# Photoroom/datago

Hardware: AMD Instinct MI355X
Metric: Mpixel/s device-resident JPEG decode+bucket-resize at 1/2/4/8 MI355X (higher is better)
Workload: dtype u8

## Files before the change

### datago_amd/csrc/kernels.hip

```cpp
#include <hip/hip_runtime.h>

#include "dg_destuff.h"
#include "dg_entropy.h"
#include "dg_pixel.h"
#include "dg_plane.h"
#include "kernels.h"

#pragma clang fp contract(off)

namespace dg {


__device__ __forceinline__ void load_tables(HuffTable *tabs, const HuffTable *pool, const ImageDesc &im) {
  const int words = (int)(sizeof(HuffTable) / 4);
  const int ns = im.nslots;
  for (int i = threadIdx.x; i < ns * words; i += blockDim.x) {
    int s = i / words, w = i - s * words;
    ((uint32_t *)&tabs[s])[w] = ((const uint32_t *)&pool[im.hslot[s]])[w];
  }
}

__device__ __forceinline__ uint32_t xcd_remap(uint32_t b, uint32_t n) {
  const uint32_t per = n >> 3, rem = n & 7, x = b & 7, l = b >> 3;
  return x * per + (x < rem ? x : rem) + l;
// ... 1020 lines not shown
    return (my * im.mcux + mx) * im.bpm + im.cfirst[c] + vy * chc + hx;
  };
  u32x4 r0 = {0, 0, 0, 0}, r1 = {0, 0, 0, 0};
  if (v0) r0 = *(const DG_GLOBAL u32x4 *)(coef + (size_t)block_index(bx0) * 64 + lane * 8);
  if (v1) r1 = *(const DG_GLOBAL u32x4 *)(coef + (size_t)block_index(bx1) * 64 + lane * 8);
  const DG_GLOBAL uint16_t *q = gp<const uint16_t>((uint64_t)(uintptr_t)qpool[im.qpool[c]].q);
  int32_t qc[8];
#pragma unroll
  for (int r = 0; r < 8; r++) qc[r] = q[r * 8 + lane];
  int32_t *bv0 = blkv + slot * LD, *bv1 = blkv + (slot + 32) * LD;
  {
    int16_t a[8], b[8];
    __builtin_memcpy(a, &r0, 16);
    __builtin_memcpy(b, &r1, 16);
#pragma unroll
    for (int i = 0; i < 8; i++) {
      const int n = kZigzagToNatural[lane * 8 + i];
      const int e = (n >> 3) * RS + (n & 7);
      bv0[e] = a[i];
      bv1[e] = b[i];
    }
  }
  __syncthreads();
  const bool zune = im.sem != 0;
  {
    int32_t v0[8], v1[8], w0[8], w1[8];
#pragma unroll
    for (int r = 0; r < 8; r++) {
      v0[r] = __mul24(bv0[r * RS + lane], qc[r]);
      v1[r] = __mul24(bv1[r * RS + lane], qc[r]);
    }
    idct_col(zune, v0, w0);
    idct_col(zune, v1, w1);
    __syncthreads();
#pragma unroll
    for (int r = 0; r < 8; r++) {
      bv0[r * RS + lane] = w0[r];
      bv1[r * RS + lane] = w1[r];
    }
  }
  __syncthreads();
  const uint32_t pst = cbw * 8;
  DG_GLOBAL uint8_t *plane = gp<uint8_t>(im.plane[c]) + (size_t)(by * 8 + lane) * pst;
  const bool rec = plane_is_rec(im, c);
  uint32_t pv[2][8];
#pragma unroll
  for (int h = 0; h < 2; h++) {
    const int32_t *w = (h ? bv1 : bv0) + lane * RS;
    const bool v = h ? v1 : v0;
    int32_t row[8];
    uint32_t px[8];
#pragma unroll
    for (int i = 0; i < 8; i++) row[i] = w[i];
    idct_row(zune, row, px);
    if (rec) {
      crec_clamp((int32_t)crec_lim(im, c) - 1 - (int32_t)((h ? bx1 : bx0) * 8), px, pv[h]);
      continue;
    }
    const uint32_t lo = pack4(px[0], px[1], px[2], px[3]), hi = pack4(px[4], px[5], px[6], px[7]);
    if (v) *(DG_GLOBAL u32x2 *)(plane + (size_t)(h ? bx1 : bx0) * 8) = u32x2{lo, hi};
  }
  if (!rec) return;
  __shared__ uint8_t efirst[kIdctBlocks * 8], elast[kIdctBlocks * 8];
#pragma unroll
  for (int h = 0; h < 2; h++) {
    const int i = slot + 32 * h;
    efirst[i * 8 + lane] = (uint8_t)pv[h][0];
    elast[i * 8 + lane] = (uint8_t)pv[h][7];
  }
  __syncthreads();
  DG_GLOBAL uint8_t *rrow = crec_row(im, c, by * 8 + lane);
#pragma unroll
  for (int h = 0; h < 2; h++) {
    if (!(h ? v1 : v0)) continue;
    const int i = slot + 32 * h;
    const uint32_t bx = h ? bx1 : bx0;
    const bool in_l = i > 0, in_r = i + 1 < (int)kIdctBlocks && bx + 1 < cbw;
    const uint32_t l = in_l ? elast[(i - 1) * 8 + lane] : pv[h][0];
    const uint32_t r = in_r ? efirst[(i + 1) * 8 + lane] : pv[h][7];
    store_crec_pair(rrow, bx, cbw, pv[h], l, r, in_l || bx == 0, in_r || bx + 1 == cbw);
  }
}

struct IdctLoc {
  uint32_t c, by, bx, bidx;
  bool v;
};
__device__ __forceinline__ bool idct_t_locate(const ImageDesc &im, uint32_t item, IdctLoc &L) {
  uint32_t c = 0;
  for (; c < im.ncomp; c++) {
    const uint32_t ck = (im.cbw[c] + kIdctBlocks - 1) / kIdctBlocks;
    const uint32_t n = im.cbh[c] * ck;
    if (item < n) break;
    item -= n;
  }
  if (c >= im.ncomp) return false;
  const uint32_t ck = (im.cbw[c] + kIdctBlocks - 1) / kIdctBlocks;
  const uint32_t by = item / ck, chunk = item - by * ck;
  const uint32_t cbw = im.cbw[c];
  const uint32_t bx = chunk * kIdctBlocks + threadIdx.x;
  const uint32_t chc = im.ch[c];
  uint32_t bidx;
  if (im.ncomp == 1) {
    bidx = by * cbw + bx;
  } else {
    const uint32_t my = by / im.cv[c], vy = by - my * im.cv[c];
    const uint32_t mx = chc == 1 ? bx : chc == 2 ? bx >> 1 : bx / chc, hx = bx - mx * chc;
    bidx = (my * im.mcux + mx) * im.bpm + im.cfirst[c] + vy * chc + hx;
  }
  L.c = c;
  L.by = by;
  L.bx = bx;
  L.v = bx < cbw;
  L.bidx = L.v ? bidx : 0u;
  return true;
}

__device__ __forceinline__ uint32_t idct_t_parts(const ImageDesc &im, const IdctLoc &L) {
  if (!L.v) return 0u;
  if (!im.ccnt) return 0xFFu;
  return gp<const uint8_t>(im.ccnt)[L.bidx];
}

__device__ __forceinline__ void idct_t_item(const ImageDesc &im, const IdctLoc &L, const u32x4 w[8],
                                            const QuantTable *__restrict__ qpool);

__global__ __launch_bounds__(64) void k_idct_t(const ImageDesc *__restrict__ imgs, const WgItem *__restrict__ list,
                                              const QuantTable *__restrict__ qpool) {
  const WgItem it = list[blockIdx.x];
  const ImageDesc &im = imgs[it.image];
  IdctLoc L;
  bool ok = idct_t_locate(im, it.item0, L);
  uint32_t np = ok ? idct_t_parts(im, L) : 0u;
#pragma nounroll
  for (uint32_t k = 0; k < kIdctItemStride && ok; k++) {
    u32x4 w[8];
    const DG_GLOBAL u32x4 *src = (const DG_GLOBAL u32x4 *)(gp<const int16_t>(im.coef) + (size_t)L.bidx * 64);
#pragma unroll
    for (uint32_t i = 0; i < 8; i++) w[i] = (np >> i) & 1u ? src[i] : u32x4{0, 0, 0, 0};
    IdctLoc N;
    const bool nok = k + 1 < kIdctItemStride && idct_t_locate(im, it.item0 + k + 1, N);
    const uint32_t nnp = nok ? idct_t_parts(im, N) : 0u;
    idct_t_item(im, L, w, qpool);
    L = N;
    ok = nok;
    np = nnp;
  }
}

__device__ __forceinline__ void idct_t_item(const ImageDesc &im, const IdctLoc &L, const u32x4 w[8],
                                            const QuantTable *__restrict__ qpool) {
  const uint32_t c = L.c, by = L.by, bx = L.bx;
  const bool v = L.v;
  const uint32_t lane = threadIdx.x, cbw = im.cbw[c];
  const bool zune = im.sem != 0;
  const DG_GLOBAL uint16_t *q = gp<const uint16_t>((uint64_t)(uintptr_t)qpool[im.qpool[c]].q);
  int32_t x[64];
  {
#pragma unroll
    for (int k = 0; k < 64; k++) {
      const uint32_t word = w[k >> 3][(k >> 1) & 3];
      const int32_t z = (int32_t)(int16_t)(k & 1 ? word >> 16 : word & 0xFFFFu);
      const int nat = kZigzagToNatural[k];
      x[nat] = __mul24(z, (int32_t)q[nat]);
    }
  }
#pragma unroll
  for (int col = 0; col < 8; col++) {
    int32_t in[8], o[8];
#pragma unroll
    for (int r = 0; r < 8; r++) in[r] = x[r * 8 + col];
    idct_col(zune, in, o);
#pragma unroll
    for (int r = 0; r < 8; r++) x[r * 8 + col] = o[r];
  }
  const bool rec = plane_is_rec(im, c);
  const int32_t e = rec ? (int32_t)crec_lim(im, c) - 1 - (int32_t)(bx * 8) : 7;
  DG_GLOBAL uint8_t *plane = gp<uint8_t>(im.plane[c]);
#pragma unroll
  for (int r = 0; r < 8; r++) {
    uint32_t px[8];
    idct_row(zune, x + r * 8, px);
    const uint32_t y = by * 8 + (uint32_t)r;
    if (!rec) {
      if (v)
        *(DG_GLOBAL u32x2 *)(plane + (size_t)y * (cbw * 8) + bx * 8) =
            u32x2{pack4(px[0], px[1], px[2], px[3]), pack4(px[4], px[5], px[6], px[7])};
      continue;
    }
    uint32_t vv[8];
    crec_clamp(e, px, vv);
    const uint32_t l = (uint32_t)__shfl_up((int)vv[7], 1), rr = (uint32_t)__shfl_down((int)vv[0], 1);
    if (v) {
      const bool have_l = lane > 0 || bx == 0, have_r = (lane + 1 < 64u && bx + 1 < cbw) || bx + 1 == cbw;
      store_crec_pair(crec_row(im, c, y), bx, cbw, vv, lane > 0 ? l : vv[0], bx + 1 < cbw ? rr : vv[7], have_l,
                      have_r);
    }
  }
}


__global__ __launch_bounds__(256) void k_idct_list(const ImageDesc *__restrict__ imgs,
                                                   const QuantTable *__restrict__ qpool,
                                                   const BatchFlags *__restrict__ flags) {
  constexpr int LD = 72, RS = 9;
  __shared__ int32_t blkv[32 * LD];
  const uint32_t n = flags->idct_late < flags->idct_cap ? flags->idct_late : flags->idct_cap;
  const DG_GLOBAL uint32_t *list = gp<const uint32_t>(flags->idct_list);
  const int t = threadIdx.x, slot = t >> 3, lane = t & 7;
  int32_t *bv = blkv + slot * LD;
  for (uint32_t base = blockIdx.x * 32; base < n; base += gridDim.x * 32) {
    const uint32_t e = base + (uint32_t)slot;
    const bool act = e < n;
    const uint32_t ii = act ? list[2 * e] : 0u, idx = act ? list[2 * e + 1] : 0u;
    const ImageDesc &im = imgs[ii];
    uint32_t c = 0, by = 0, bx = 0;
    if (act) block_pos(im, idx, c, by, bx);
    if (act) {
      const u32x4 r0 = *(const DG_GLOBAL u32x4 *)(gp<const int16_t>(im.coef) + (size_t)idx * 64 + lane * 8);
      int16_t a[8];
      __builtin_memcpy(a, &r0, 16);
#pragma unroll
      for (int i = 0; i < 8; i++) {
        const int nn = kZigzagToNatural[lane * 8 + i];
        bv[(nn >> 3) * RS + (nn & 7)] = a[i];
      }
    }
    __syncthreads();
    int32_t w[8];
    if (act) {
      const DG_GLOBAL uint16_t *q = gp<const uint16_t>((uint64_t)(uintptr_t)qpool[im.qpool[c]].q);
      int32_t v[8];
#pragma unroll
      for (int r = 0; r < 8; r++) v[r] = bv[r * RS + lane] * (int32_t)q[r * 8 + lane];
      idct_col(im.sem != 0, v, w);
    }
    __syncthreads();
    if (act) {
#pragma unroll
      for (int r = 0; r < 8; r++) bv[r * RS + lane] = w[r];
    }
    __syncthreads();
    if (act) {
      int32_t row[8];
      uint32_t px[8];
#pragma unroll
      for (int i = 0; i < 8; i++) row[i] = bv[lane * RS + i];
      idct_row(im.sem != 0, row, px);
      store_plane_row8(im, c, by * 8 + lane, bx, px);
    }
    __syncthreads();
  }
}


template <class P>
__device__ __forceinline__ void upsample8(P pl, uint32_t stride, uint32_t hr, uint32_t vr,
                                          uint32_t dsw, uint32_t dsh, uint32_t x0, uint32_t y, int32_t o[8],
                                          bool rec = false) {
  if (rec) {
    const uint32_t c0 = x0 >> 1;
    int32_t cs[6];
    const bool fancy = dsw > 2;
    if (vr == 1 || !fancy) {
      load_crec6(pl, stride, vr == 1 ? y : y >> 1, c0, cs);
      if (!fancy) {
#pragma unroll
        for (int k = 0; k < 8; k++) o[k] = cs[1 + (k >> 1)];
        return;
      }
#pragma unroll
      for (int k = 0; k < 4; k++) {
        const int32_t a = cs[k + 1] * 3;
        o[2 * k] = (a + cs[k] + 1) >> 2;
        o[2 * k + 1] = (a + cs[k + 2] + 2) >> 2;
      }
      return;
    }
    const uint32_t r = y >> 1;
// ... 2006 lines not shown
```

### datago_amd/csrc/dg_entropy.h

```cpp
#pragma once
#include "dg_pixel.h"
#include "dg_plane.h"
#include "dg_types.h"

namespace dg {

DG_HD int32_t huff_extend(int32_t v, int32_t s) { return v < (1 << (s - 1)) ? v - (1 << s) + 1 : v; }

DG_HD uint32_t bswap32(uint32_t x) {
  return (x >> 24) | ((x >> 8) & 0xFF00u) | ((x << 8) & 0xFF0000u) | (x << 24);
}

DG_HD uint32_t ds_word_index(uint32_t w, uint32_t lsw) {
  const uint32_t s = w >> lsw, j = w & ((1u << lsw) - 1u);
  return ((((s >> 6) << lsw) + j) << 6) + (s & 63u);
}
DG_HD uint64_t ds_words_alloc(uint32_t nsub, uint32_t lsw) {
  const uint32_t margin = ((1024u >> 5) >> lsw) + 2u;
  return ((uint64_t)((nsub + margin + 63u) / 64u) << lsw) * 64;
}

constexpr uint32_t kBwBuf = 6;

struct BitWin {
  const DG_GLOBAL uint32_t *w;
  uint64_t win;
  uint32_t base;
  uint32_t lsw;
  uint32_t nbuf;
  uint32_t buf[kBwBuf];
};

DG_HD uint32_t bw_word(const BitWin &b, uint32_t i) { return b.w[ds_word_index(i, b.lsw)]; }

DG_HD void bw_fill(BitWin &b) {
  const uint32_t nw = (b.base >> 5) + 2u;
#pragma unroll
  for (uint32_t k = 0; k < kBwBuf; k++) b.buf[k] = bw_word(b, nw + k);
  b.nbuf = kBwBuf;
}

DG_HD void bw_init(BitWin &b, const DG_GLOBAL uint8_t *stream, uint32_t lsw, uint32_t pos) {
  b.w = (const DG_GLOBAL uint32_t *)stream;
  b.lsw = lsw;
  uint32_t i = pos >> 5;
  b.base = i << 5;
  b.win = ((uint64_t)bswap32(bw_word(b, i)) << 32) | bswap32(bw_word(b, i + 1));
  bw_fill(b);
}

DG_HD void bw_refill(BitWin &b) {
#if defined(DG_DEVICE)
  if (__ballot(b.nbuf == 0u)) bw_fill(b);
#else
  if (b.nbuf == 0u) bw_fill(b);
#endif
}

DG_HD uint32_t bw_peek(const BitWin &b, uint32_t pos) { return (uint32_t)((b.win << (pos - b.base)) >> 32); }

DG_HD void bw_shift(BitWin &b, uint32_t pos) {
  const bool adv = pos - b.base >= 32u;
  b.win = adv ? (b.win << 32) | bswap32(b.buf[0]) : b.win;
  b.base += adv ? 32u : 0u;
#pragma unroll
  for (uint32_t k = 0; k + 1 < kBwBuf; k++) b.buf[k] = adv ? b.buf[k + 1] : b.buf[k];
  b.nbuf -= adv ? 1u : 0u;
}

DG_HD void bw_seek(BitWin &b, uint32_t pos) {
  if (pos - b.base >= 32u) bw_init(b, (const DG_GLOBAL uint8_t *)b.w, b.lsw, pos);
}

template <class T>
DG_HD uint32_t huff_lookup(const T &t, uint32_t bits) {
  uint32_t e = t.lut[bits >> (32 - kLutBits)];
  if (!(e & 0x8000u) && e) return e;
  if (e & 0x8000u) {
    uint32_t e2 = t.sub[e & (kMaxSubTables - 1)][(bits >> (32 - 16)) & ((1u << kSubBits) - 1)];
    return e2 ? e2 : (16u << 8);
  }
  uint32_t pk = bits >> 16;
  for (int32_t l = kLutBits + 1; l <= 16; l++)
    if (pk < t.lim[l]) return ((uint32_t)l << 8) | t.vals[(t.valoff[l] + (int32_t)(pk >> (16 - l))) & 255];
  return 16u << 8;
}

template <class T>
DG_HD uint32_t huff_decode(const T &t, uint32_t bits) {
  const uint32_t e = t.lut[bits >> (32 - kLutBits)];
  if (e != 0u && !(e & 0x8000u)) return e;
  return huff_lookup(t, bits);
}

DG_HD int32_t huff_value(uint32_t bits, uint32_t len, uint32_t size) {
  const uint32_t raw = (uint32_t)((uint64_t)(bits << len) >> (32u - size));
  const uint32_t half = (1u << size) >> 1;
  return raw < half ? (int32_t)raw - (int32_t)((1u << size) - 1u) : (int32_t)raw;
}

DG_HD uint32_t huff_next_z(uint32_t z, uint32_t sym) {
  const uint32_t size = sym & 15u, run = sym >> 4;
  const uint32_t zac = (size == 0u && run != 15u) ? 64u : z + run + 1u;
  return z == 0u ? 1u : zac;
}

#ifndef DG_MULTI_BITS
#define DG_MULTI_BITS 11
#endif
constexpr uint32_t kMultiBits = DG_MULTI_BITS;
constexpr uint32_t kMultiLuts = 3;

template <class TAB>
DG_HD uint32_t multi_entry(const TAB &t, uint32_t pfx) {
  const uint32_t bits = pfx << (32u - kMultiBits);
  uint32_t o = 0, adv = 0, eob = 0;
  while (o < kMultiBits) {
    const uint32_t e = huff_lookup(t, bits << o);
    const uint32_t len = e >> 8, sym = e & 0xFFu, size = sym & 15u, run = sym >> 4;
    if (len == 0u || len >= 16u || o + len + size > kMultiBits) break;
    if (size == 0u && run != 15u) {
      o += len;
      eob = 1;
      break;
    }
    const uint32_t nadv = adv + (size == 0u ? 16u : run + 1u);
    if (nadv > 64u) break;
    adv = nadv;
    o += len + size;
    if (adv == 64u) break;
  }
  return o | (adv << 4) | (eob << 11);
}

DG_HD uint32_t multi_next_z(uint32_t m, uint32_t z) {
  const uint32_t c = m & 15u, adv = (m >> 4) & 127u, eob = (m >> 11) & 1u;
  const bool ok = c != 0u && z != 0u && (eob ? z + adv < 64u : z + adv <= 64u);
  return ok ? (eob ? 64u : z + adv) : 0xFFFFFFFFu;
}

#if defined(DG_STEP_STATS) && !defined(DG_DEVICE)
struct StepStats {
  uint64_t lead_steps, range_steps, chained, over32;
};
inline StepStats g_step_stats = {0, 0, 0, 0};
#define DG_STEP_STAT(field, n) (g_step_stats.field += (n))
#else
#define DG_STEP_STAT(field, n) ((void)0)
#endif

#ifndef DG_CHAIN_DC
#define DG_CHAIN_DC 1
#endif
DG_HD void multi_chain(const uint16_t *mt, uint32_t mi, uint32_t bits, uint32_t chain, bool open, uint32_t ev,
                       uint32_t &used, uint32_t &pos, uint32_t &zn) {
#pragma unroll
  for (uint32_t x = 0; x < 3u; x++) {
    if (x >= chain) break;
    const uint32_t bx = used < 32u ? bits << used : 0u;
    const uint32_t m = (open && mi != 3u) ? (uint32_t)mt[(mi << kMultiBits) | (bx >> (32u - kMultiBits))] : 0u;
    const uint32_t c = m & 15u;
    const uint32_t zx = multi_next_z(m, zn);
    const bool tk = zx != 0xFFFFFFFFu && pos + c <= ev && used + c <= 32u;
    pos += tk ? c : 0u;
    used += tk ? c : 0u;
    zn = tk ? zx : zn;
    DG_STEP_STAT(chained, tk ? 1u : 0u);
  }
}

template <int NC>
struct RangeAccN {
  uint32_t out;
  uint32_t m, n;
  int32_t dc[NC];
};
using RangeAcc = RangeAccN<3>;
template <class T>
struct NoDeduce {
  typedef T type;
};

struct WriteCtxBase {
  int16_t *blk;
  uint32_t sw = 0;
  DG_GLOBAL int16_t *coef;
  uint32_t seg, nin;
  uint32_t blocks_per_seg, total_blocks;
  int32_t cur;
  uint32_t zs;
#if defined(DG_DEVICE)
  DG_GLOBAL uint8_t *cnt = nullptr;
  int16_t *wave_blk;
  uint32_t stride;
  uint32_t *tab;
  const ImageDesc *im;
  const int32_t *qt;
  const uint8_t *n2z;
  BatchFlags *flags;
  uint32_t img;
#endif
};
template <int NC>
struct WriteCtxN : WriteCtxBase {
  int32_t pred[NC];
};
using WriteCtx = WriteCtxN<3>;

DG_HD int32_t wc_index(const WriteCtxBase &w, uint32_t in_seg) {
  if (w.blocks_per_seg && in_seg >= w.blocks_per_seg) return -1;
  uint64_t g = (uint64_t)(w.blocks_per_seg ? w.seg : 0) * w.blocks_per_seg + in_seg;
  return g < w.total_blocks ? (int32_t)g : -1;
}

template <bool MS>
DG_HD int32_t wc_index_ms(const ImageDesc &im, const WriteCtxBase &w, uint32_t in_seg) {
  const int32_t g = wc_index(w, in_seg);
  if (MS && g >= 0 && im.ms.role == kMsScan) return (int32_t)ms_index(im.ms, (uint32_t)g);
  return g;
}

DG_HD void wc_begin(WriteCtxBase &w, int32_t idx, uint32_t zs) {
  w.cur = idx;
  w.zs = zs;
#if defined(DG_DEVICE)
  u32x4 *p = (u32x4 *)w.blk;
  const u32x4 zero = {0u, 0u, 0u, 0u};
#pragma unroll
  for (int i = 0; i < 8; i++) p[i] = zero;
#else
  for (int i = 0; i < 64; i++) w.blk[i] = 0;
#endif
}

DG_HD void wc_flush(WriteCtxBase &w, uint32_t ze) {
  if (w.cur < 0) return;
  DG_GLOBAL int16_t *dst = w.coef + (size_t)w.cur * 64;
  if (w.zs == 0 && ze == 64) {
#if defined(DG_DEVICE)
    const u32x4 *s4 = (const u32x4 *)w.blk;
    DG_GLOBAL u32x4 *d4 = (DG_GLOBAL u32x4 *)dst;
#pragma unroll
    for (int i = 0; i < 8; i++) d4[i] = s4[i ^ (w.sw >> 3)];
#else
    for (int i = 0; i < 64; i++) dst[i] = w.blk[i ^ w.sw];
#endif
  } else {
    for (uint32_t i = w.zs; i < ze; i++) dst[i] = w.blk[i ^ w.sw];
  }
#if defined(DG_DEVICE)
  if (w.cnt) w.cnt[w.cur] = 0xFFu;
#endif
  w.cur = -1;
}

#if defined(DG_DEVICE)
__device__ __forceinline__ void wc_list_late(WriteCtxBase &w, int32_t idx) {
  if (!w.im || idx < 0) return;
  const uint32_t e = atomicAdd(&w.flags->idct_late, 1u);
  if (e < w.flags->idct_cap) {
    uint32_t *l = (uint32_t *)(uintptr_t)w.flags->idct_list;
    l[2 * e] = w.img;
    l[2 * e + 1] = (uint32_t)idx;
  }
}

__device__ __forceinline__ void wc_coop_flush(WriteCtxBase &w, bool pending) {
  const uint64_t pm = __ballot(pending);
  if (!pm) return;
  const uint64_t am = __ballot(1);
  if (pending) {
    const uint32_t rank = __builtin_amdgcn_mbcnt_hi((uint32_t)(pm >> 32), __builtin_amdgcn_mbcnt_lo((uint32_t)pm, 0u));
    w.tab[rank] = __lane_id();
    w.tab[64 + rank] = (uint32_t)w.cur;
  }
  __builtin_amdgcn_wave_barrier();
  const uint32_t wr = __builtin_amdgcn_mbcnt_hi((uint32_t)(am >> 32), __builtin_amdgcn_mbcnt_lo((uint32_t)am, 0u));
  const uint32_t na = (uint32_t)__popcll(am), nb = (uint32_t)__popcll(pm), nc = 8u * nb;
  const u32x4 zero = {0u, 0u, 0u, 0u};
  if (w.im && na >= 8) {
    const ImageDesc &im = *w.im;
    const bool zune = im.sem != 0;
    const uint32_t groups = na >> 3, g = wr >> 3, part = wr & 7u;
    for (uint32_t k0 = 0; k0 < nb; k0 += groups) {
      const uint32_t k = k0 + g;
      const bool act = g < groups && k < nb;
      const int32_t idx = act ? (int32_t)w.tab[64 + k] : -1;
      const uint32_t own = act ? w.tab[k] & 255u : 0u;
      int16_t *b = w.wave_blk + own * w.stride;
      const uint32_t osw = w.stride == 64u ? ((own >> 1) & 7u) << 3 : 0u;
      const bool live = act && idx >= 0;
      uint32_t c = 0, by = 0, bx = 0;
      if (live) block_pos(im, (uint32_t)idx, c, by, bx);
      int32_t ws[8];
      if (live) {
        int32_t v[8];
#pragma unroll
        for (int r = 0; r < 8; r++) v[r] = (int32_t)b[w.n2z[r * 8 + part] ^ osw] * w.qt[c * 64 + r * 8 + part];
        idct_col(zune, v, ws);
      }
      __builtin_amdgcn_wave_barrier();
      if (live) {
#pragma unroll
        for (int r = 0; r < 8; r++) b[r * 8 + part] = (int16_t)ws[r];
      }
      __builtin_amdgcn_wave_barrier();
      if (act) {
        u32x4 *row4 = (u32x4 *)b + part;
        if (live) {
          const u32x4 rv = *row4;
          int16_t h[8];
          __builtin_memcpy(h, &rv, 16);
          int32_t row[8];
          uint32_t px[8];
#pragma unroll
          for (int i = 0; i < 8; i++) row[i] = h[i];
          idct_row(zune, row, px);
          store_plane_row8(im, c, by * 8 + part, bx, px);
        }
        *row4 = zero;
      }
      __builtin_amdgcn_wave_barrier();
    }
    return;
  }
  for (uint32_t c = wr; c < nc; c += na) {
    const uint32_t k = c >> 3, part = c & 7u;
    const int32_t idx = (int32_t)w.tab[64 + k];
    const uint32_t own = w.tab[k] & 255u;
    u32x4 *src = (u32x4 *)(w.wave_blk + own * w.stride) + (w.stride == 64u ? part ^ ((own >> 1) & 7u) : part);
    const u32x4 v = *src;
    const bool nz = (v.x | v.y | v.z | v.w) != 0u;
    if (idx >= 0 && (nz || !w.cnt)) *(DG_GLOBAL u32x4 *)(w.coef + (size_t)idx * 64 + part * 8) = v;
    if (w.cnt && nz) atomicOr(&w.tab[k], 256u << part);
    *src = zero;
    if (part == 0) wc_list_late(w, idx);
  }
  __builtin_amdgcn_wave_barrier();
  if (w.cnt && wr < nb) {
    const int32_t idx = (int32_t)w.tab[64 + wr];
    if (idx >= 0) w.cnt[idx] = (uint8_t)(w.tab[wr] >> 8);
  }
  __builtin_amdgcn_wave_barrier();
}

__device__ __forceinline__ void wc_flush_zero(WriteCtxBase &w, uint32_t ze) {
  wc_flush(w, ze);
  u32x4 *p = (u32x4 *)w.blk;
  const u32x4 zero = {0u, 0u, 0u, 0u};
#pragma unroll
  for (int i = 0; i < 8; i++) p[i] = zero;
}
#endif

template <bool COOP>
DG_HD void wc_end_block(WriteCtxBase &w, bool &pending) {
#if defined(DG_DEVICE)
  if (COOP) {
    if (w.zs == 0) {
      pending = true;
    } else {
      const int32_t idx = w.cur;
      wc_flush_zero(w, 64);
      wc_list_late(w, idx);
    }
    return;
  }
#endif
  (void)pending;
  wc_flush(w, 64);
}
template <bool COOP>
DG_HD void wc_partial(WriteCtxBase &w, uint32_t ze) {
#if defined(DG_DEVICE)
  if (COOP) {
    wc_flush_zero(w, ze);
    return;
  }
#endif
  wc_flush(w, ze);
}

struct StageCtx {
  DG_GLOBAL uint32_t *base;
  uint32_t on;
  uint32_t n, started;
  uint32_t g0, g1, g2, g3;
};
DG_HD uint32_t stage_coef(uint32_t zz, uint32_t j, int32_t v) {
  return (zz << 25) | ((j & 0x1FFFu) << 12) | ((uint32_t)v & 0xFFFu);
}
DG_HD uint32_t stage_marker(uint32_t owned, uint32_t z, uint32_t j) {
  return 0x80000000u | (owned << 30) | ((z & 63u) << 24) | ((j & 0x1FFFu) << 11);
}
DG_HD DG_GLOBAL uint32_t *stage_range(uint64_t stage, uint32_t cap, uint32_t s) {
  return (DG_GLOBAL uint32_t *)(uintptr_t)stage + ((((size_t)(s >> 6) * cap) << 6) + (s & 63u)) * 4;
}
DG_HD void stage_push(StageCtx &c, uint32_t e) {
  const uint32_t k = c.n & 3u;
  c.g0 = k == 0 ? e : c.g0;
  c.g1 = k == 1 ? e : c.g1;
  c.g2 = k == 2 ? e : c.g2;
  c.g3 = k == 3 ? e : c.g3;
  c.n++;
  if (k == 3) {
    DG_GLOBAL uint32_t *p = c.base + (size_t)((c.n >> 2) - 1) * 256;
// ... 153 lines not shown
  if (WRITE) {
    w->cur = -1;
    if (z > 0) wc_begin(*w, w->nin > 0 ? wc_index_ms<MS>(im, *w, w->nin - 1) : -1, z);
  }
  auto next_event = [&]() -> uint32_t {
    uint32_t e = a1 < mpos ? a1 : mpos;
    return (k < nck && cpos < e) ? cpos : e;
  };
  const bool multi = !WRITE && !stage && mt != nullptr;
  uint32_t mi = 3u;
  auto block_tables = [&](const TAB *&tdc, const TAB *&tac) {
    tdc = &tabs[(slotmap >> ((comp << 1) << 2)) & 15u];
    tac = &tabs[(slotmap >> (((comp << 1) | 1u) << 2)) & 15u];
    mi = multi ? (acm >> (2u * comp)) & 3u : 3u;
  };
  const TAB *tdc, *tac;
  block_tables(tdc, tac);
  uint32_t ev = next_event();
  for (;;) {
#if defined(DG_DEVICE)
    if (WRITE && COOP) {
      wc_coop_flush(*w, pending);
      pending = false;
    }
#endif
    if (pos >= ev) {
      if (pos >= mpos) {
        bool owned = mpos < a1;
        if (WRITE && z > 0) wc_partial<COOP>(*w, z);
        if (stage) stage_push(*stg, stage_marker(owned ? 1u : 0u, z, stg->started));
        pos = mpos;
        r = 0;
        z = 0;
        comp = cbits & 3u;
        block_tables(tdc, tac);
        if (owned) {
          acc.m++;
          acc.n = 0;
          setn(acc.dc, 0);
          if (WRITE) {
            w->seg++;
            w->nin = 0;
            setn(w->pred, 0);
          }
        }
        midx++;
        mpos = midx < im.nmk ? mk[midx] : kInf;
        bw_seek(b, pos);
      }
      if (k < nck && cpos < a1 && pos >= cpos) {
        uint32_t rel = pos - cpos;
        uint32_t st = pack_state(rel > 255 ? 255 : rel, r, z);
        DG_GLOBAL CkptN<NC> &c = ck[k];
        if (merge && c.st == st) {
          if (c.m) {
            acc.m += c.m;
            acc.n = c.n;
            cpyn<NC>(acc.dc, c.dc);
          } else {
            acc.n += c.n;
            accn<NC>(acc.dc, c.dc);
          }
          acc.out = old_out;
          merged = true;
          break;
        }
        c.st = st;
        c.m = acc.m;
        c.n = acc.n;
        cpyn<NC>(c.dc, acc.dc);
        k++;
        cpos += kCkptBits;
      }
      if (pos >= a1) break;
      ev = next_event();
    }
    bw_refill(b);
    const uint32_t bits = bw_peek(b, pos);
    const bool isdc = (z == 0);
    const uint32_t e = huff_decode(*(isdc ? tdc : tac), bits);
    const uint32_t len = e >> 8, sym = e & 0xFFu;
    const uint32_t size = sym & 15u;
    const uint32_t run = isdc ? 0u : (sym >> 4);
    const int32_t v = huff_value(bits, len, size);
    uint32_t zm = 0xFFFFFFFFu, mc = 0;
    if (!WRITE) {
      const uint32_t m = (mi != 3u && !isdc) ? (uint32_t)mt[(mi << kMultiBits) | (bits >> (32u - kMultiBits))] : 0u;
      mc = m & 15u;
      zm = pos + mc <= ev ? multi_next_z(m, z) : 0xFFFFFFFFu;
    }
    const bool take_m = zm != 0xFFFFFFFFu;
    const uint32_t p0 = pos;
    pos += take_m ? mc : len + size;
    const int32_t vdc = isdc ? v : 0;
    acc.n += isdc ? 1u : 0u;
    addn(acc.dc, comp, vdc);
    if (stage) {
      if (isdc) {
        stg->started++;
        if (v) stage_push(*stg, stage_coef(0, stg->started, v));
      } else if (size && z + run < 64) {
        stage_push(*stg, stage_coef(z + run, stg->started, v));
      }
    }
    if (WRITE) {
      addn(w->pred, comp, vdc);
      if (isdc) {
        if (COOP) {
          w->cur = wc_index_ms<MS>(im, *w, w->nin);
          w->zs = 0;
        } else {
          wc_begin(*w, wc_index_ms<MS>(im, *w, w->nin), 0);
        }
        w->nin++;
      }
      const uint32_t zz = z + run;
      if (isdc || (size && zz < 64u)) w->blk[zz ^ w->sw] = (int16_t)(isdc ? seln(w->pred, comp) : v);
    }
    uint32_t zn = take_m ? zm : huff_next_z(z, sym);
    if (pair && !stage && (WRITE || !take_m)) {
      uint32_t used = len + size;
      bool open = isdc || !(size == 0u && run != 15u);
#pragma unroll
      for (uint32_t x = 0; x < 3u; x++) {
        if (x >= pair) break;
        const uint32_t bx = used < 32u ? bits << used : 0u;
        const uint32_t ex = huff_decode(*tac, bx);
        const uint32_t lx = ex >> 8, sx = ex & 0xFFu, zx = sx & 15u;
        const bool tk = open && zn < 64u && pos < ev && used + lx + zx <= 32u;
        if (tk) {
          if (WRITE) {
            const uint32_t zz2 = zn + (sx >> 4);
            if (zx && zz2 < 64u) w->blk[zz2 ^ w->sw] = (int16_t)huff_value(bx, lx, zx);
          }
          pos += lx + zx;
          used += lx + zx;
          zn = huff_next_z(zn, sx);
        }
        open = tk && !(zx == 0u && (sx >> 4) != 15u);
      }
    }
    if (!WRITE && chain) {
      uint32_t used = pos - p0;
      multi_chain(mt, mi, bits, chain, DG_CHAIN_DC || !isdc, ev, used, pos, zn);
    }
    if (!WRITE) {
      DG_STEP_STAT(range_steps, 1u);
      DG_STEP_STAT(over32, pos - p0 > 32u ? 1u : 0u);
    }
    bw_shift(b, pos);
    const bool bend = zn >= 64u;
    if (WRITE && bend) wc_end_block<COOP>(*w, pending);
    z = bend ? 0u : zn;
    r = bend ? (r + 1u == bpm ? 0u : r + 1u) : r;
    comp = (cbits >> (2u * r)) & 3u;
    block_tables(tdc, tac);
  }
  if (WRITE && z > 0) wc_partial<COOP>(*w, z);
  if (stage) stage_finish(*stg);
  if (!merged) {
    uint32_t rel = pos - a1;
    acc.out = pack_state(rel > 255 ? 255 : rel, r, z);
  }
  for (uint32_t j = 0; j < k; j++) {
    DG_GLOBAL CkptN<NC> &c = ck[j];
    if (acc.m > c.m) {
      c.m = acc.m - c.m;
      c.n = acc.n;
      cpyn<NC>(c.dc, acc.dc);
    } else {
      c.m = 0;
      c.n = acc.n - c.n;
      rsubn<NC>(c.dc, acc.dc);
    }
  }
}

template <class TAB>
struct SyncChain {
  BitWin b;
  uint32_t pos, r, z, comp, mi, ev;
  uint32_t phase;
  uint32_t a0, a1, mpos, midx, k, cpos, nck;
  uint32_t in;
  const TAB *tdc, *tac;
  RangeAcc acc;
  DG_GLOBAL Ckpt *ck;
};

template <class TAB>
DG_HD void schain_tables(SyncChain<TAB> &c, const ImageDesc &im, const TAB *tabs, const uint16_t *mt, uint32_t acm) {
  c.tdc = &tabs[(im.slotmap >> ((c.comp << 1) << 2)) & 15u];
  c.tac = &tabs[(im.slotmap >> (((c.comp << 1) | 1u) << 2)) & 15u];
  c.mi = mt ? (acm >> (2u * c.comp)) & 3u : 3u;
}

template <class TAB>
DG_HD void schain_range(SyncChain<TAB> &c, const ImageDesc &im, const TAB *tabs, const DG_GLOBAL uint8_t *stream,
                        const DG_GLOBAL uint32_t *mk, const uint16_t *mt, uint32_t acm, bool fresh) {
  c.phase = 1;
  c.acc.m = 0;
  c.acc.n = 0;
  c.acc.dc[0] = c.acc.dc[1] = c.acc.dc[2] = 0;
  c.r = st_r(c.in);
  c.z = st_z(c.in);
  if (c.a0 >= im.ds_bits) {
    c.acc.out = pack_state(0, 0, 0);
    c.phase = 2;
    c.ev = kInf;
    c.comp = (im.comp_bits >> (2 * c.r)) & 3u;
    schain_tables(c, im, tabs, mt, acm);
    if (fresh) {
      c.pos = 0;
      bw_init(c.b, stream, im.ds_lsw, 0);
    }
    return;
  }
  c.pos = c.a0 + st_rel(c.in);
  c.mpos = im.nmk ? first_marker(mk, im.nmk, c.a0, c.midx) : kInf;
  if (fresh) bw_init(c.b, stream, im.ds_lsw, c.pos < c.a1 ? c.pos : c.a0);
  c.comp = (im.comp_bits >> (2 * c.r)) & 3u;
  schain_tables(c, im, tabs, mt, acm);
  c.k = 0;
  c.cpos = c.a0 + kCkptBits;
  const uint32_t e = c.a1 < c.mpos ? c.a1 : c.mpos;
  c.ev = (c.k < c.nck && c.cpos < e) ? c.cpos : e;
}

template <class TAB>
DG_HD void schain_begin(SyncChain<TAB> &c, const ImageDesc &im, const TAB *tabs, const DG_GLOBAL uint8_t *stream,
                        const DG_GLOBAL uint32_t *mk, uint32_t s, uint32_t lead, bool active, DG_GLOBAL Ckpt *ck,
// ... 183 lines not shown
```

Baseline: 140,500.

## Hoist per-image IDCT geometry into scalar registers and cache quant table

The k_idct_t kernel now reads the image descriptor through the constant address space and packs each component's geometry into wave-uniform values via readfirstlane, so they sit in scalar registers. Successive work items are reached by stepping a position incrementally instead of searching again with divisions on every item. The quant table is loaded once into registers through scalar loads and reloaded only when the quant slot changes, replacing per-element global 16-bit loads. The intent is to cut vector memory traffic and integer overhead in the IDCT loop, at the cost of more registers and hand-written crec row addressing that must match crec_row.

```diff
diff --git a/datago_amd/csrc/kernels.hip b/datago_amd/csrc/kernels.hip
--- a/datago_amd/csrc/kernels.hip
+++ b/datago_amd/csrc/kernels.hip
@@ -1126,79 +1126,163 @@
   }
 }
 
-struct IdctLoc {
-  uint32_t c, by, bx, bidx;
-  bool v;
+#define DG_CONST __attribute__((address_space(4)))
+
+struct IdctComp {
+  uint32_t cbw, cbh;
+  uint32_t lim;
+  uint32_t ch, cv, cfirst;
+  bool rec;
+  uint32_t qslot;
+  uint64_t plane;
 };
-__device__ __forceinline__ bool idct_t_locate(const ImageDesc &im, uint32_t item, IdctLoc &L) {
-  uint32_t c = 0;
-  for (; c < im.ncomp; c++) {
-    const uint32_t ck = (im.cbw[c] + kIdctBlocks - 1) / kIdctBlocks;
-    const uint32_t n = im.cbh[c] * ck;
-    if (item < n) break;
+struct IdctGeo {
+  uint32_t dims[4];
+  uint32_t info[4];
+  uint64_t plane[4];
+  uint32_t qslots[2];
+  uint32_t ncomp, mcux, bpm;
+  uint64_t coef, ccnt;
+  bool zune;
+};
+struct IdctPos {
+  uint32_t c, chunk, my, vy;
+  bool ok;
+};
+
+__device__ __forceinline__ uint32_t uni(uint32_t v) { return (uint32_t)__builtin_amdgcn_readfirstlane((int)v); }
+__device__ __forceinline__ uint64_t uni64(uint64_t v) { return (uint64_t)uni((uint32_t)(v >> 32)) << 32 | uni((uint32_t)v); }
+
+template <class T>
+__device__ __forceinline__ T idct_t_pick(uint32_t c, T a0, T a1, T a2, T a3) {
+  return c >= 2 ? (c == 3 ? a3 : a2) : (c == 1 ? a1 : a0);
+}
+__device__ __forceinline__ IdctComp idct_t_comp(const IdctGeo &g, uint32_t c) {
+  IdctComp r;
+  const uint32_t dims = idct_t_pick(c, g.dims[0], g.dims[1], g.dims[2], g.dims[3]);
+  const uint32_t info = idct_t_pick(c, g.info[0], g.info[1], g.info[2], g.info[3]);
+  r.cbw = dims & 0xFFFFu;
+  r.cbh = dims >> 16;
+  r.ch = info & 7u;
+  r.cv = (info >> 3) & 7u;
+  r.cfirst = (info >> 6) & 0x1FFu;
+  r.rec = (info >> 15) & 1u;
+  r.lim = g.zune ? r.cbw * 8 : info >> 16;
+  r.qslot = ((c & 2u ? g.qslots[1] : g.qslots[0]) >> (16 * (c & 1u))) & 0xFFFFu;
+  r.plane = idct_t_pick(c, g.plane[0], g.plane[1], g.plane[2], g.plane[3]);
+  return r;
+}
+
+__device__ __forceinline__ IdctPos idct_t_locate(const IdctGeo &g, uint32_t item) {
+  IdctPos p = {0, 0, 0, 0, false};
+  for (; p.c < g.ncomp; p.c++) {
+    const IdctComp cc = idct_t_comp(g, p.c);
+    const uint32_t ck = (cc.cbw + kIdctBlocks - 1) / kIdctBlocks, n = cc.cbh * ck;
+    if (item < n) {
+      const uint32_t by = item / ck;
+      p.chunk = item - by * ck;
+      p.my = by / cc.cv;
+      p.vy = by - p.my * cc.cv;
+      p.ok = true;
+      break;
+    }
     item -= n;
   }
-  if (c >= im.ncomp) return false;
-  const uint32_t ck = (im.cbw[c] + kIdctBlocks - 1) / kIdctBlocks;
-  const uint32_t by = item / ck, chunk = item - by * ck;
-  const uint32_t cbw = im.cbw[c];
-  const uint32_t bx = chunk * kIdctBlocks + threadIdx.x;
-  const uint32_t chc = im.ch[c];
+  return p;
+}
+
+__device__ __forceinline__ void idct_t_next(const IdctGeo &g, IdctPos &p) {
+  const IdctComp cc = idct_t_comp(g, p.c);
+  if (++p.chunk < (cc.cbw + kIdctBlocks - 1) / kIdctBlocks) return;
+  p.chunk = 0;
+  if (++p.vy == cc.cv) {
+    p.vy = 0;
+    p.my++;
+  }
+  if (p.my * cc.cv + p.vy < cc.cbh) return;
+  p.my = p.vy = 0;
+  p.ok = ++p.c < g.ncomp;
+}
+
+__device__ __forceinline__ uint32_t idct_t_block(const IdctGeo &g, const IdctPos &p, bool &v) {
+  const IdctComp cc = idct_t_comp(g, p.c);
+  const uint32_t bx = p.chunk * kIdctBlocks + threadIdx.x;
+  v = p.ok && bx < cc.cbw;
   uint32_t bidx;
-  if (im.ncomp == 1) {
-    bidx = by * cbw + bx;
+  if (g.ncomp == 1) {
+    bidx = (p.my * cc.cv + p.vy) * cc.cbw + bx;
   } else {
-    const uint32_t my = by / im.cv[c], vy = by - my * im.cv[c];
+    const uint32_t chc = cc.ch;
     const uint32_t mx = chc == 1 ? bx : chc == 2 ? bx >> 1 : bx / chc, hx = bx - mx * chc;
-    bidx = (my * im.mcux + mx) * im.bpm + im.cfirst[c] + vy * chc + hx;
-  }
-  L.c = c;
-  L.by = by;
-  L.bx = bx;
-  L.v = bx < cbw;
-  L.bidx = L.v ? bidx : 0u;
-  return true;
-}
-
-__device__ __forceinline__ uint32_t idct_t_parts(const ImageDesc &im, const IdctLoc &L) {
-  if (!L.v) return 0u;
-  if (!im.ccnt) return 0xFFu;
-  return gp<const uint8_t>(im.ccnt)[L.bidx];
-}
-
-__device__ __forceinline__ void idct_t_item(const ImageDesc &im, const IdctLoc &L, const u32x4 w[8],
-                                            const QuantTable *__restrict__ qpool);
+    bidx = (p.my * g.mcux + mx) * g.bpm + cc.cfirst + p.vy * chc + hx;
+  }
+  return v ? bidx : 0u;
+}
+
+__device__ __forceinline__ uint32_t idct_t_parts(const IdctGeo &g, uint32_t bidx, bool v) {
+  if (!v) return 0u;
+  if (!g.ccnt) return 0xFFu;
+  return gp<const uint8_t>(g.ccnt)[bidx];
+}
+
+__device__ __forceinline__ void idct_t_item(const IdctGeo &g, const IdctPos &p, const u32x4 w[8], const uint32_t qw[32]);
 
 __global__ __launch_bounds__(64) void k_idct_t(const ImageDesc *__restrict__ imgs, const WgItem *__restrict__ list,
                                               const QuantTable *__restrict__ qpool) {
   const WgItem it = list[blockIdx.x];
-  const ImageDesc &im = imgs[it.image];
-  IdctLoc L;
-  bool ok = idct_t_locate(im, it.item0, L);
-  uint32_t np = ok ? idct_t_parts(im, L) : 0u;
+  const DG_CONST ImageDesc *im = (const DG_CONST ImageDesc *)(imgs + uni(it.image));
+  IdctGeo g;
+  g.ncomp = uni(im->ncomp);
+  g.mcux = uni(im->mcux);
+  g.bpm = uni(im->bpm);
+  g.coef = uni64(im->coef);
+  g.ccnt = uni64(im->ccnt);
+  g.zune = uni(im->sem) != 0;
+  const uint32_t crec = uni(im->crec);
+#pragma unroll
+  for (uint32_t j = 0; j < 4; j++) {
+    g.dims[j] = uni(im->cbw[j] | im->cbh[j] << 16);
+    g.info[j] = uni(im->ch[j] | im->cv[j] << 3 | im->cfirst[j] << 6 | ((crec >> j) & 1u) << 15 | im->cdsw[j] << 16);
+    g.plane[j] = uni64(im->plane[j]);
+  }
+  g.qslots[0] = uni(im->qpool[0] | (uint32_t)im->qpool[1] << 16);
+  g.qslots[1] = uni(im->qpool[2] | (uint32_t)im->qpool[3] << 16);
+  IdctPos p = idct_t_locate(g, uni(it.item0));
+  if (!p.ok) return;
+  bool v;
+  uint32_t bidx = idct_t_block(g, p, v);
+  uint32_t np = idct_t_parts(g, bidx, v);
+  asm volatile("" ::"v"(np));
+  uint32_t qw[32], qslot = ~0u;
 #pragma nounroll
-  for (uint32_t k = 0; k < kIdctItemStride && ok; k++) {
+  for (uint32_t k = 0; p.ok; k++) {
     u32x4 w[8];
-    const DG_GLOBAL u32x4 *src = (const DG_GLOBAL u32x4 *)(gp<const int16_t>(im.coef) + (size_t)L.bidx * 64);
+    const DG_GLOBAL u32x4 *src = (const DG_GLOBAL u32x4 *)(gp<const int16_t>(g.coef) + (size_t)bidx * 64);
 #pragma unroll
     for (uint32_t i = 0; i < 8; i++) w[i] = (np >> i) & 1u ? src[i] : u32x4{0, 0, 0, 0};
-    IdctLoc N;
-    const bool nok = k + 1 < kIdctItemStride && idct_t_locate(im, it.item0 + k + 1, N);
-    const uint32_t nnp = nok ? idct_t_parts(im, N) : 0u;
-    idct_t_item(im, L, w, qpool);
-    L = N;
-    ok = nok;
-    np = nnp;
-  }
-}
-
-__device__ __forceinline__ void idct_t_item(const ImageDesc &im, const IdctLoc &L, const u32x4 w[8],
-                                            const QuantTable *__restrict__ qpool) {
-  const uint32_t c = L.c, by = L.by, bx = L.bx;
-  const bool v = L.v;
-  const uint32_t lane = threadIdx.x, cbw = im.cbw[c];
-  const bool zune = im.sem != 0;
-  const DG_GLOBAL uint16_t *q = gp<const uint16_t>((uint64_t)(uintptr_t)qpool[im.qpool[c]].q);
+    const uint32_t slot = idct_t_comp(g, p.c).qslot;
+    if (slot != qslot) {
+      qslot = slot;
+      const DG_CONST uint32_t *q = (const DG_CONST uint32_t *)(qpool + slot);
+#pragma unroll
+      for (int i = 0; i < 32; i++) qw[i] = q[i];
+    }
+    IdctPos n = p;
+    idct_t_next(g, n);
+    n.ok = n.ok && k + 1 < kIdctItemStride;
+    bidx = idct_t_block(g, n, v);
+    np = idct_t_parts(g, bidx, v);
+    asm volatile("" ::: "memory");
+    idct_t_item(g, p, w, qw);
+    p = n;
+  }
+}
+
+__device__ __forceinline__ void idct_t_item(const IdctGeo &g, const IdctPos &p, const u32x4 w[8], const uint32_t qw[32]) {
+  const IdctComp cc = idct_t_comp(g, p.c);
+  const uint32_t by = p.my * cc.cv + p.vy, lane = threadIdx.x, bx = p.chunk * kIdctBlocks + lane, cbw = cc.cbw;
+  const bool v = bx < cbw;
+  const bool zune = g.zune;
   int32_t x[64];
   {
 #pragma unroll
@@ -1206,7 +1290,8 @@
       const uint32_t word = w[k >> 3][(k >> 1) & 3];
       const int32_t z = (int32_t)(int16_t)(k & 1 ? word >> 16 : word & 0xFFFFu);
       const int nat = kZigzagToNatural[k];
-      x[nat] = __mul24(z, (int32_t)q[nat]);
+      const uint32_t q = nat & 1 ? qw[nat >> 1] >> 16 : qw[nat >> 1] & 0xFFFFu;
+      x[nat] = __mul24(z, (int32_t)q);
     }
   }
 #pragma unroll
@@ -1218,9 +1303,9 @@
 #pragma unroll
     for (int r = 0; r < 8; r++) x[r * 8 + col] = o[r];
   }
-  const bool rec = plane_is_rec(im, c);
-  const int32_t e = rec ? (int32_t)crec_lim(im, c) - 1 - (int32_t)(bx * 8) : 7;
-  DG_GLOBAL uint8_t *plane = gp<uint8_t>(im.plane[c]);
+  const bool rec = cc.rec;
+  const int32_t e = rec ? (int32_t)cc.lim - 1 - (int32_t)(bx * 8) : 7;
+  DG_GLOBAL uint8_t *plane = gp<uint8_t>(cc.plane);
 #pragma unroll
   for (int r = 0; r < 8; r++) {
     uint32_t px[8];
@@ -1237,8 +1322,8 @@
     const uint32_t l = (uint32_t)__shfl_up((int)vv[7], 1), rr = (uint32_t)__shfl_down((int)vv[0], 1);
     if (v) {
       const bool have_l = lane > 0 || bx == 0, have_r = (lane + 1 < 64u && bx + 1 < cbw) || bx + 1 == cbw;
-      store_crec_pair(crec_row(im, c, y), bx, cbw, vv, lane > 0 ? l : vv[0], bx + 1 < cbw ? rr : vv[7], have_l,
-                      have_r);
+      store_crec_pair(plane + (size_t)y * (cbw * 16), bx, cbw, vv, lane > 0 ? l : vv[0], bx + 1 < cbw ? rr : vv[7],
+                      have_l, have_r);
     }
   }
 }
```

After: 140,800, median of 2. Within noise of the previous version (+0.2%).

## Branchless write-path Huffman pair decode and ballot-based coop flush masks

Applied to the files above, without the earlier changes.

Reworks the WRITE (coefficient emit) path of the entropy decoder. The multi-symbol pair loop becomes branch-free with a remaining-bits budget, uses a cheaper 32-bit sign-extend helper and selects the DC predictor without an indexed lookup. The cooperative block flush gains a fast path for multiple-of-8 active lanes that builds nonzero-part masks with a wave ballot instead of LDS atomics. Step-count stats are extended for the write path. The aim is less divergence and fewer atomics, at the cost of more code paths to keep correct.

```diff
diff --git a/datago_amd/csrc/dg_entropy.h b/datago_amd/csrc/dg_entropy.h
--- a/datago_amd/csrc/dg_entropy.h
+++ b/datago_amd/csrc/dg_entropy.h
@@ -97,6 +97,13 @@
   const uint32_t raw = (uint32_t)((uint64_t)(bits << len) >> (32u - size));
   const uint32_t half = (1u << size) >> 1;
   return raw < half ? (int32_t)raw - (int32_t)((1u << size) - 1u) : (int32_t)raw;
+}
+
+DG_HD int32_t huff_value32(uint32_t bits, uint32_t len, uint32_t size) {
+  const uint32_t t = bits << len;
+  const uint32_t raw = (t >> 1) >> (31u - size);
+  const uint32_t ones = (1u << size) - 1u;
+  return (int32_t)raw - (int32_t)((t & 0x80000000u) ? 0u : ones);
 }
 
 DG_HD uint32_t huff_next_z(uint32_t z, uint32_t sym) {
@@ -142,6 +149,7 @@
 #if defined(DG_STEP_STATS) && !defined(DG_DEVICE)
 struct StepStats {
   uint64_t lead_steps, range_steps, chained, over32;
+  uint64_t wsteps, wslot[3], wbend, wover32;
 };
 inline StepStats g_step_stats = {0, 0, 0, 0};
 #define DG_STEP_STAT(field, n) (g_step_stats.field += (n))
@@ -254,6 +262,20 @@
   w.cur = -1;
 }
 
+DG_HD uint32_t flush_part_mask(uint64_t am, uint64_t bm, uint32_t lane) {
+  if (am == ~(uint64_t)0) return (uint32_t)(bm >> (lane & 56u)) & 0xFFu;
+  uint64_t a = am >> lane;
+  const uint64_t b = bm >> lane;
+  uint32_t mask = 0;
+#pragma unroll
+  for (uint32_t p = 0; p < 8u; p++) {
+    const uint64_t low = a & (0 - a);
+    mask |= (b & low) ? 1u << p : 0u;
+    a ^= low;
+  }
+  return mask;
+}
+
 #if defined(DG_DEVICE)
 __device__ __forceinline__ void wc_list_late(WriteCtxBase &w, int32_t idx) {
   if (!w.im || idx < 0) return;
@@ -262,6 +284,27 @@
     uint32_t *l = (uint32_t *)(uintptr_t)w.flags->idct_list;
     l[2 * e] = w.img;
     l[2 * e + 1] = (uint32_t)idx;
+  }
+}
+
+template <bool FULL>
+__device__ __forceinline__ void wc_flush_groups(WriteCtxBase &w, uint64_t am, uint32_t wr, uint32_t na, uint32_t nc) {
+  const uint32_t lane = __lane_id(), part = wr & 7u;
+  const u32x4 zero = {0u, 0u, 0u, 0u};
+  for (uint32_t c = wr; c < nc; c += na) {
+    const uint32_t k = c >> 3;
+    const int32_t idx = (int32_t)w.tab[64 + k];
+    const uint32_t own = w.tab[k];
+    u32x4 *src = (u32x4 *)(w.wave_blk + own * w.stride) + (w.stride == 64u ? part ^ ((own >> 1) & 7u) : part);
+    const u32x4 v = *src;
+    const bool nz = (v.x | v.y | v.z | v.w) != 0u;
+    if (idx >= 0 && (nz || !w.cnt)) *(DG_GLOBAL u32x4 *)(w.coef + (size_t)idx * 64 + part * 8) = v;
+    *src = zero;
+    if (w.cnt) {
+      const uint64_t bm = __ballot(nz);
+      const uint32_t mask = FULL ? (uint32_t)(bm >> (lane & 56u)) & 0xFFu : flush_part_mask(am, bm, lane);
+      if (part == 0u && idx >= 0) w.cnt[idx] = (uint8_t)mask;
+    }
   }
 }
 
@@ -322,6 +365,12 @@
       }
       __builtin_amdgcn_wave_barrier();
     }
+    return;
+  }
+  if ((na & 7u) == 0u) {
+    if (am == ~(uint64_t)0) wc_flush_groups<true>(w, am, wr, na, nc);
+    else wc_flush_groups<false>(w, am, wr, na, nc);
+    __builtin_amdgcn_wave_barrier();
     return;
   }
   for (uint32_t c = wr; c < nc; c += na) {
@@ -641,7 +690,7 @@
     const uint32_t len = e >> 8, sym = e & 0xFFu;
     const uint32_t size = sym & 15u;
     const uint32_t run = isdc ? 0u : (sym >> 4);
-    const int32_t v = huff_value(bits, len, size);
+    const int32_t v = WRITE ? huff_value32(bits, len, size) : huff_value(bits, len, size);
     uint32_t zm = 0xFFFFFFFFu, mc = 0;
     if (!WRITE) {
       const uint32_t m = (mi != 3u && !isdc) ? (uint32_t)mt[(mi << kMultiBits) | (bits >> (32u - kMultiBits))] : 0u;
@@ -674,29 +723,47 @@
         w->nin++;
       }
       const uint32_t zz = z + run;
-      if (isdc || (size && zz < 64u)) w->blk[zz ^ w->sw] = (int16_t)(isdc ? seln(w->pred, comp) : v);
+      const int32_t q0 = w->pred[0], q1 = w->pred[1], q2 = w->pred[2], q3 = w->pred[NC - 1];
+      const int32_t pv = comp == 0u ? q0 : (comp == 1u ? q1 : ((NC == 4 && comp == 3u) ? q3 : q2));
+      const int16_t cv = (int16_t)(isdc ? pv : v);
+      if (isdc || (size && zz < 64u)) w->blk[zz ^ w->sw] = cv;
     }
     uint32_t zn = take_m ? zm : huff_next_z(z, sym);
     if (pair && !stage && (WRITE || !take_m)) {
       uint32_t used = len + size;
-      bool open = isdc || !(size == 0u && run != 15u);
-#pragma unroll
-      for (uint32_t x = 0; x < 3u; x++) {
-        if (x >= pair) break;
-        const uint32_t bx = used < 32u ? bits << used : 0u;
-        const uint32_t ex = huff_decode(*tac, bx);
-        const uint32_t lx = ex >> 8, sx = ex & 0xFFu, zx = sx & 15u;
-        const bool tk = open && zn < 64u && pos < ev && used + lx + zx <= 32u;
-        if (tk) {
-          if (WRITE) {
-            const uint32_t zz2 = zn + (sx >> 4);
-            if (zx && zz2 < 64u) w->blk[zz2 ^ w->sw] = (int16_t)huff_value(bx, lx, zx);
+      if (WRITE) {
+        uint32_t evr = (zn < 64u && ev > p0) ? ev - p0 : 0u;
+#pragma unroll
+        for (uint32_t x = 0; x < 3u; x++) {
+          if (x >= pair) break;
+          const uint32_t bx = bits << (used & 31u);
+          const uint32_t ex = huff_decode(*tac, bx);
+          const uint32_t lx = ex >> 8, sx = ex & 0xFFu, zx = sx & 15u, rx = sx >> 4, cx = lx + zx;
+          const bool tk = used < evr && used + cx <= 32u;
+          const uint32_t zz2 = zn + rx;
+          if (tk && zx && zz2 < 64u) w->blk[zz2 ^ w->sw] = (int16_t)huff_value32(bx, lx, zx);
+          used += tk ? cx : 0u;
+          zn = tk ? ((zx == 0u && rx != 15u) ? 64u : zz2 + 1u) : zn;
+          evr = (tk && zn < 64u) ? evr : 0u;
+          DG_STEP_STAT(wslot[x], tk ? 1u : 0u);
+        }
+        pos = p0 + used;
+      } else {
+        bool open = isdc || !(size == 0u && run != 15u);
+#pragma unroll
+        for (uint32_t x = 0; x < 3u; x++) {
+          if (x >= pair) break;
+          const uint32_t bx = used < 32u ? bits << used : 0u;
+          const uint32_t ex = huff_decode(*tac, bx);
+          const uint32_t lx = ex >> 8, sx = ex & 0xFFu, zx = sx & 15u;
+          const bool tk = open && zn < 64u && pos < ev && used + lx + zx <= 32u;
+          if (tk) {
+            pos += lx + zx;
+            used += lx + zx;
+            zn = huff_next_z(zn, sx);
           }
-          pos += lx + zx;
-          used += lx + zx;
-          zn = huff_next_z(zn, sx);
+          open = tk && !(zx == 0u && (sx >> 4) != 15u);
         }
-        open = tk && !(zx == 0u && (sx >> 4) != 15u);
       }
     }
     if (!WRITE && chain) {
@@ -706,6 +773,10 @@
     if (!WRITE) {
       DG_STEP_STAT(range_steps, 1u);
       DG_STEP_STAT(over32, pos - p0 > 32u ? 1u : 0u);
+    } else {
+      DG_STEP_STAT(wsteps, 1u);
+      DG_STEP_STAT(wbend, zn >= 64u ? 1u : 0u);
+      DG_STEP_STAT(wover32, pos - p0 > 32u ? 1u : 0u);
     }
     bw_shift(b, pos);
     const bool bend = zn >= 64u;
```

After: 142,000 before, 143,400 after (median of 6 runs). No clear change (+1.0%).
